# ultravideo/kvazaar

Measured on AMD Instinct MI355X. Metric: CTUs/s (all-intra ultrafast hot path), higher is better.
Workload: dtype u8/i16 (f64 RD costs)

## Files before the change

### include/kvz_hip_dev.h

```cpp
#ifndef KVZ_HIP_DEV_H_
#define KVZ_HIP_DEV_H_

#include "kvz_hip_types.h"

#ifdef __cplusplus
extern "C" {
#endif

void *kvz_hip_dev_alloc(size_t bytes);
void  kvz_hip_dev_free(void *p);
void  kvz_hip_dev_upload(void *dev_dst, const void *host_src, size_t bytes);
void  kvz_hip_dev_download(void *host_dst, const void *dev_src, size_t bytes);
void  kvz_hip_dev_sync(void);
void  kvz_hip_dev_copy(void *dev_dst, const void *dev_src, size_t bytes);
void  kvz_hip_dev_timer_start(void);
float kvz_hip_dev_timer_stop(void);

int  kvz_hip_dev_sad_nxn(int n, const uint8_t *a, const uint8_t *b, int count, uint32_t *out);
int  kvz_hip_dev_satd_nxn(int n, const uint8_t *a, const uint8_t *b, int count, uint32_t *out);

int  kvz_hip_dev_transform(int kind, const int16_t *in, int16_t *tmp, int16_t *out, int count, int use_matrix_cores);

int  kvz_hip_dev_angular_pred(int log2_width, int mode, const uint8_t *ref_above, const uint8_t *ref_left, int count, uint8_t *out);

int  kvz_hip_dev_intra_select(int log2w, int nblk, const uint32_t *raw, const int8_t *preds, const double *mode_bits, int count, int32_t *winner);

void kvz_hip_dev_deblock_frames(uint8_t *frames, int width, int height, int n_frames, const uint8_t *cu_depth, int qp, int beta_offset_div2,
                                int tc_offset_div2);

typedef struct kvz_hip_cu_dbk {
  uint8_t type;
  uint8_t depth, tr_depth, part_size;
  uint8_t cbf_y;
  uint8_t mv_dir;
  int8_t  mv_ref[2];
  int16_t ref_id[2];
  int16_t mv[2][2];
} kvz_hip_cu_dbk;
void kvz_hip_dev_deblock_frames_inter(uint8_t *frames, int width, int height, int n_frames, const kvz_hip_cu_dbk *info, int qp, int beta_offset_div2,
                                      int tc_offset_div2, int slice_is_b);

int  kvz_hip_dev_loop_filters_inter(const uint8_t *src, uint8_t *rec, int width, int height, int n_pictures, const kvz_hip_cu_dbk *info, int qp, int slice_is_b, int deblock,
                                    int beta_offset_div2, int tc_offset_div2, int sao, int no_wpp, kvz_hip_sao_params *luma, kvz_hip_sao_params *chroma, uint8_t *merge);

int  kvz_hip_dev_sad_surface(const uint8_t *cur, const uint8_t *ref, int width, int height, int bw, int range, const int16_t *blk_xy, int count,
                             uint32_t *out);

typedef struct kvz_hip_fme_pu {
// ... 98 lines not shown
```

### kvazaar_amd/csrc/kvz_ctu.hpp

```cpp
#pragma once
#include <type_traits>
#include "../../include/kvz_hip_types.h"
#include "kvz_ops.hpp"
#include "kvz_rdoq.hpp"
#include "kvz_recon.hpp"
#include "kvz_residual.hpp"
#include "kvz_select.hpp"

namespace kvz {

#define KVZ_CTU_THREADS 128
#ifdef KVZ_HOSTSIM
#define KVZ_FOR_THREADS(tid) for (int tid = 0; tid < KVZ_CTU_THREADS; ++tid)
#ifdef KVZ_HOSTSIM_COUNT_SYNCS
static unsigned long long g_kvz_syncs;
#define KVZ_SYNC() (++g_kvz_syncs)
#else
#define KVZ_SYNC()
#endif
#define KVZ_LDS_ADD(p, v) (*(p) += (v))
#else
#define KVZ_FOR_THREADS(tid) for (int tid = (threadIdx.x + lane_rot) & (KVZ_CTU_THREADS - 1), once_ = 1; once_; once_ = 0)
#define KVZ_SYNC() __syncthreads()
#define KVZ_LDS_ADD(p, v) atomicAdd((p), (v))
#endif
#ifdef KVZ_HOSTSIM
#define KVZ_WAVE_SYNC()
#else
#define KVZ_WAVE_SYNC() do { __builtin_amdgcn_fence(__ATOMIC_RELEASE, "wavefront"); __builtin_amdgcn_wave_barrier(); __builtin_amdgcn_fence(__ATOMIC_ACQUIRE, "wavefront"); } while (0)
#endif

#ifdef KVZ_HOSTSIM
#define KVZ_TOGETHER(...)
#else
#define KVZ_TG1(v) "+v"(v)
#define KVZ_TG_PICK(_1, _2, _3, _4, _5, _6, _7, _8, _9, _10, NAME, ...) NAME
#define KVZ_TG_2(a, b) KVZ_TG1(a), KVZ_TG1(b)
#define KVZ_TG_5(a, b, c, d, e) KVZ_TG1(a), KVZ_TG1(b), KVZ_TG1(c), KVZ_TG1(d), KVZ_TG1(e)
#define KVZ_TG_10(a, b, c, d, e, f, g, h, i, j) KVZ_TG_5(a, b, c, d, e), KVZ_TG_5(f, g, h, i, j)
#define KVZ_TOGETHER(...) asm volatile("" : KVZ_TG_PICK(__VA_ARGS__, KVZ_TG_10, _9, _8, _7, _6, KVZ_TG_5, _4, _3, KVZ_TG_2, _1)(__VA_ARGS__))
#endif

KVZ_DEV void block_add(u32 *dst, u32 v)
{
#ifdef KVZ_HOSTSIM
  *dst += v;
#else
  const int x = row16_sum((int)v);
  const u32 total = (u32)(__builtin_amdgcn_readlane(x, 15) + __builtin_amdgcn_readlane(x, 31) + __builtin_amdgcn_readlane(x, 47) + __builtin_amdgcn_readlane(x, 63));
  if ((threadIdx.x & 63) == 0 && total) atomicAdd(dst, total);
#endif
}
// ... 789 lines not shown
        const int c = g < ny ? 0 : 1, i = g - (c == 0 ? 0 : ny);
        const int l2 = c ? log2w_c : log2w_y, n = 2 * (1 << l2) + 1, side = i >= n, k = side ? i - n : i;
        int qx, qy, dv;
        const bool have = ref_coords(l2, c, x, y, side, k, avail_top, avail_left, &qx, &qy);
        const lds_off off = rec_off(lv, c, qx, qy, &dv);
        s->ref[c][side][k] = have ? base[off] : (u8)128;
        if (c) s->ref[2][side][k] = have ? base[off + dv] : (u8)128;
      }
    }
    KVZ_SYNC();
    KVZ_FOR_THREADS(tid) {
      if (luma) {
        const int n = 2 * (1 << log2w_y) + 1;
        for (int i = tid; i < 2 * n; i += KVZ_CTU_THREADS) {
          const int side = i >= n, k = side ? i - n : i;
          const u8 *r = s->ref[0][side];
          u8 v;
          if (k == 0) v = (u8)((s->ref[0][1][1] + 2 * s->ref[0][1][0] + s->ref[0][0][1] + 2) / 4);
          else if (k == n - 1) v = r[k];
          else v = (u8)((r[k - 1] + 2 * r[k] + r[k + 1] + 2) / 4);
          s->fref[side][k] = v;
        }
      }
      const int c = tid - (KVZ_CTU_THREADS - 3);
      if (c >= 0 && ((c == 0 && luma) || (c > 0 && chroma))) {
        const int l2 = c ? log2w_c : log2w_y, w = 1 << l2;
#ifdef KVZ_HOSTSIM
        s->dcval[c] = (u8)dc_value(l2, s->ref[c][0], s->ref[c][1]);
#else
        u32 sum = 0;
        for (int i = 0; i < w; i += 4) {
          u32 a, b;
          __builtin_memcpy(&a, &s->ref[c][0][1 + i], 4);
          __builtin_memcpy(&b, &s->ref[c][1][1 + i], 4);
          sum = __builtin_amdgcn_sad_u8(a, 0u, sum);
          sum = __builtin_amdgcn_sad_u8(b, 0u, sum);
        }
        s->dcval[c] = (u8)((sum + w) >> (l2 + 1));
#endif
      }
    }
    KVZ_SYNC();
    KVZ_PROF(KVZ_P_REFS);
  }

  KVZ_DEV u8 predict_pixel(int log2w, int mode, int c, int x, int y) const
  {
// ... 504 lines not shown
  KVZ_DEV void transform_big(int l2, i16 *x, bool inverse, int tid, int c) const
  {
#ifndef KVZ_HOSTSIM
    if ((tid >> 6) != (c & 1)) return;
    if (l2 == 5) mfma_transform_block<32>(x, x, inverse, tb, tid & 63);
    else mfma_transform_block<16>(x, x, inverse, tb, tid & 63);
#else
    if (tid != 0) return;
    const int n = 1 << l2;
    i16 tmp[32 * 32];
    for (int pass = 0; pass < 2; pass++) {
      const i16 *src = pass == 0 ? x : tmp;
      i16 *dst = pass == 0 ? tmp : x;
      const int shift = inverse ? (pass == 0 ? 7 : 12) : (pass == 0 ? l2 - 1 : l2 + 6);
      for (int e = 0; e < n * n; e++) {
        const int hi = e >> l2, lo = e & (n - 1);
        dst[e] = inverse ? inv_point(n, [&](int k) { return dct_at(l2, k, lo); }, src, hi, n, shift) : fwd_point(n, [&](int i) { return dct_at(l2, hi, i); }, src, lo << l2, shift);
      }
    }
#endif
  }

  enum RowPlan { ROWS_CU8, ROWS_W16, ROWS_W32_Y, ROWS_W32_C };
  KVZ_DEV void plane_sums(RowPlan plan, int tid, int c, u32 v, bool packed, int base) const
  {
#ifdef KVZ_HOSTSIM
    (void)tid;
    if (c < 0) return;
    if (packed && plan != ROWS_CU8) { s->acc[3 + c] += v & 0xffffffu; s->acc[6 + c] += v >> 24; }
    else s->acc[base + c] += v;
#else
    (void)c;
    if ((plan == ROWS_W16 || plan == ROWS_W32_C) && tid >= 64) return;
    const int x = row16_sum((int)v);
    const u32 r0 = (u32)__builtin_amdgcn_readlane(x, 15), r1 = (u32)__builtin_amdgcn_readlane(x, 31), r2 = (u32)__builtin_amdgcn_readlane(x, 47), r3 = (u32)__builtin_amdgcn_readlane(x, 63);
    if ((tid & 63) != 0) return;
    if (plan == ROWS_CU8) {
      if (tid < 64) s->acc[base] += r0 + r1 + r2 + r3;
      else { s->acc[base + 1] += r0; s->acc[base + 2] += r1; }
      return;
    }
    auto put = [&](int plane, u32 a, u32 b) {
      if (packed) {
        const u32 ws = (a & 0xffffffu) + (b & 0xffffffu), n = (a >> 24) + (b >> 24);
        if (n) { atomicAdd(&s->acc[3 + plane], ws); atomicAdd(&s->acc[6 + plane], n); }
        else if (ws) atomicAdd(&s->acc[3 + plane], ws);
      } else if (a + b) atomicAdd(&s->acc[base + plane], a + b);
    };
    if (plan == ROWS_W16) { put(0, r0, r1); put(1, r2, 0); put(2, r3, 0); }
    else if (plan == ROWS_W32_Y) { put(0, r0, r1); put(0, r2, r3); }
    else { put(1, r0, r1); put(2, r2, r3); }
#endif
  }
  KVZ_DEV void finish_planes(int lv, int xl, int yl, int depth, int c0, int c1, bool packed) const
  {
    for (int c = c0; c < c1; c++) {
      u32 n = s->acc[6 + c];
      if (packed) { const u32 pk = s->acc[3 + c]; n = pk >> 24; s->acc[3 + c] = pk & 0xffffffu; s->acc[6 + c] = n; }
      if (NXN && lv == 4) { if (c == 0) rl->pu_cbf[rl->n_pu] = n != 0; else rl->pu_cbf_c[c - 1] = n != 0; }
      else {
        CtuCu *cu = &s->cu[lv][(yl >> 3) * 8 + (xl >> 3)];
        cbf_clear(&cu->cbf, depth, c);
        if (n) cbf_set(&cu->cbf, depth, c);
      }
    }
  }
  KVZ_DEV void hide_signs(int tid, int log2y, int log2c, int scan, const i16 *cf_y, i16 *lv_y, const i16 *cf_u, i16 *lv_u, const i16 *cf_v, i16 *lv_v) const
  {
    if constexpr (SH) {
      const int wv = tid >> 6, lane = tid & 63;
      const int c = wv == 0 ? 0 : 1 + (lane >> 4), i = wv == 0 ? lane : (lane & 15), l2 = wv == 0 ? log2y : log2c, groups = 1 << (2 * l2 - 4);
      const bool live = c < 3 && i < groups;
      const i16 *cf = c == 0 ? cf_y : (c == 1 ? cf_u : cf_v);
      i16 *lv = c == 0 ? lv_y : (c == 1 ? lv_u : lv_v);
// ... 14 lines not shown
      const bool first_visited = ((behind >> i) >> 1) == 0;
#endif
      if (any) {
        auto at = [&](int n) { const int r = scan_in_group(scan, n); return base + ((r >> 2) << l2) + (r & 3); };
        const SignHideChange ch = sign_hide_group([&](int n) { return (int)lv[at(n)]; }, [&](int n) { return (int)cf[at(n)]; }, s->qs[l2 - 2][c ? 1 : 0], first_visited);
        if (ch.pos >= 0) { const int o = at(ch.pos); lv[o] = (i16)sign_hide_apply(lv[o], cf[o], ch.step); }
      }
    }
  }
  KVZ_DEV void recon_cu8(int lv, const TuSet &t, int depth, int mode)
  {
    const int xl = t.x - cx, yl = t.y - cy;
    const CandView cv = cand_view(lv);
#define KVZ_CU8_STAGE(body) KVZ_FOR_THREADS(tid) { if (tid < 64) { body(std::true_type(), tid); } else if (tid < 96) { body(std::false_type(), tid); } }
#define KVZ_CU8_ROLE(tid)                                                                                               \
    constexpr bool LUMA = decltype(luma)::value;                                                                        \
    constexpr int l2 = LUMA ? 3 : 2, n = 1 << l2, sh = LUMA ? 0 : 1;                                                    \
    const int c = LUMA ? 0 : ((tid) < 80 ? 1 : 2), e = LUMA ? (tid) : ((tid) & 15);                                     \
    (void)sh; (void)n; (void)c; (void)e
    KVZ_FOR_THREADS(tid) {
      if (tid < 2) s->acc[3 * tid] = 0;
      if (tid >= 64 && tid < 68) s->acc[1 + (tid - 64) + ((tid - 64) >> 1)] = 0;
    }
    auto stage1 = [&](auto luma, int tid) {
      KVZ_CU8_ROLE(tid);
      const int px = e & (n - 1), py = e >> l2;
      const u8 p = predict_pixel(l2, mode, c, px, py);
      cv.at(c, (xl >> sh) + px, (yl >> sh) + py) = p;
      tbuf(t, 0, c)[e] = (i16)((int)*org_at(c, (xl >> sh) + px, (yl >> sh) + py) - (int)p);
    };
    KVZ_CU8_STAGE(stage1)
    KVZ_WAVE_SYNC();
    KVZ_PROF(KVZ_P_RPRED);
    auto stage2 = [&](auto luma, int tid) {
      KVZ_CU8_ROLE(tid);
      const int k = e >> l2, j = e & (n - 1);
      constexpr int shift = l2 - 1, add = 1 << (shift - 1);
      const i16 *src = tbuf(t, 0, c);
      int a = 0;
#pragma unroll
      for (int i = 0; i < n; i++) a += dct_at(l2, k, i) * (int)src[(j << l2) + i];
      tbuf(t, 1, c)[e] = (i16)((a + add) >> shift);
    };
    KVZ_CU8_STAGE(stage2)
    KVZ_WAVE_SYNC();
    KVZ_PROF(KVZ_P_FDCT);
    const bool hide = hide_on();
    KVZ_FOR_THREADS(tid) {
      u32 packed = 0;
      auto stage3 = [&](auto luma, int tid_) {
        KVZ_CU8_ROLE(tid_);
        const int k = e >> l2, j = e & (n - 1);
        constexpr int shift = l2 + 6, add = 1 << (shift - 1);
        const i16 *src = tbuf(t, 1, c);
        int a = 0;
#pragma unroll
        for (int i = 0; i < n; i++) a += dct_at(l2, k, i) * (int)src[(j << l2) + i];
        const int cf = (i16)((a + add) >> shift);
        const QuantScalars q = s->qs[l2 - 2][LUMA ? 0 : 1];
        ListFactor f{ 0, 0 };
        if constexpr (LISTS) f = factor_at(c, l2, e);
        const int level = LISTS ? quant_level(cf, q, f.fwd) : quant_level(cf, q);
        levels_lds(lv, c)[e] = (i16)level;
        if constexpr (SH) { if (hide) { tbuf(t, 0, c)[e] = (i16)cf; return; } }
        tbuf(t, 0, c)[e] = LISTS ? dequant_level(level, q, f.inv) : dequant_level(level, q);
        packed = level_cost(level, m->coeff_weights).word();
      };
      if (tid < 64) stage3(std::true_type(), tid); else if (tid < 96) stage3(std::false_type(), tid);
      if (!hide) plane_sums(ROWS_CU8, tid, tid < 64 ? 0 : (tid < 80 ? 1 : (tid < 96 ? 2 : -1)), packed, true, 3);
    }
    if constexpr (SH) {
      if (hide) {
        KVZ_WAVE_SYNC();
        KVZ_FOR_THREADS(tid) { hide_signs(tid, 3, 2, intra_scan_order(mode, depth), tbuf(t, 0, 0), levels_lds(lv, 0), tbuf(t, 0, 1), levels_lds(lv, 1), tbuf(t, 0, 2), levels_lds(lv, 2)); }
        KVZ_WAVE_SYNC();
        KVZ_FOR_THREADS(tid) {
          u32 packed = 0;
          auto stage3b = [&](auto luma, int tid_) {
            KVZ_CU8_ROLE(tid_);
            const int level = levels_lds(lv, c)[e];
            tbuf(t, 0, c)[e] = dequant_level(level, s->qs[l2 - 2][LUMA ? 0 : 1]);
            packed = level_cost(level, m->coeff_weights).word();
          };
          if (tid < 64) stage3b(std::true_type(), tid); else if (tid < 96) stage3b(std::false_type(), tid);
          plane_sums(ROWS_CU8, tid, tid < 64 ? 0 : (tid < 80 ? 1 : (tid < 96 ? 2 : -1)), packed, true, 3);
        }
      }
    }
    KVZ_WAVE_SYNC();
    KVZ_PROF(KVZ_P_QUANT);
    auto stage4 = [&](auto luma, int tid) {
      KVZ_CU8_ROLE(tid);
      if (s->acc[3 + c] >> 24) {
        const int j = e >> l2, i = e & (n - 1);
        constexpr int shift = 7, add = 1 << (shift - 1);
        const i16 *src = tbuf(t, 0, c);
        int a = 0;
#pragma unroll
        for (int k = 0; k < n; k++) a += dct_at(l2, k, i) * (int)src[(k << l2) + j];
        tbuf(t, 1, c)[e] = (i16)iclip(-32768, 32767, (a + add) >> shift);
      }
    };
    KVZ_CU8_STAGE(stage4)
    KVZ_WAVE_SYNC();
    KVZ_PROF(KVZ_P_IDCT);
    KVZ_FOR_THREADS(tid) {
      u32 ssd = 0;
      auto stage5 = [&](auto luma, int tid_) {
        KVZ_CU8_ROLE(tid_);
        u8 *rp = &cv.at(c, (xl >> sh) + (e & (n - 1)), (yl >> sh) + (e >> l2));
        int v = *rp;
        if (s->acc[3 + c] >> 24) {
          const int j = e >> l2, i = e & (n - 1);
          constexpr int shift = 12, add = 1 << (shift - 1);
          const i16 *src = tbuf(t, 1, c);
          int a = 0;
#pragma unroll
          for (int k = 0; k < n; k++) a += dct_at(l2, k, i) * (int)src[(k << l2) + j];
          const i16 res = (i16)iclip(-32768, 32767, (a + add) >> shift);
          v = recon_sample(v, res);
          *rp = (u8)v;
        }
        ssd = sq_err(*org_at(c, (xl >> sh) + (e & (n - 1)), (yl >> sh) + (e >> l2)), v);
      };
      if (tid < 64) stage5(std::true_type(), tid); else if (tid < 96) stage5(std::false_type(), tid);
      plane_sums(ROWS_CU8, tid, tid < 64 ? 0 : (tid < 80 ? 1 : (tid < 96 ? 2 : -1)), ssd, false, 0);
    }
    KVZ_SYNC();
    KVZ_FOR_THREADS(tid) {
      if (tid == 0) finish_planes(lv, xl, yl, depth, 0, 3, true);
    }
    if (cabac_on()) KVZ_SYNC();
    KVZ_PROF(KVZ_P_RECON);
#undef KVZ_CU8_ROLE
#undef KVZ_CU8_STAGE
  }

  KVZ_DEV void rdoq_unit(int tid, int lv, const TuSet &t, bool chroma, int depth, int mode) const
  {
#ifdef KVZ_HOSTSIM
    const int wv = tid == 0 ? 0 : (tid == 64 ? 1 : -1), lane = 0;
#else
    const int wv = tid >> 6, lane = tid & 63;
#endif
    for (int c = 0; c < (chroma ? 3 : 1); c++) {
      if (wv != (c ? 1 : 0)) continue;
      RdoqWaveArgs ra;
      ra.ptab = (KVZ_LDS_PTR(const i32))rl->ptab; ra.coef = (KVZ_LDS_PTR(const i16))tbuf(t, 0, c); ra.dest = (KVZ_LDS_PTR(i16))levels_lds(lv, c);
      ra.diag8 = (KVZ_LDS_PTR(const u8))rl->diag8; ra.lambda = m->lambda; ra.qp = m->qp; ra.log2w = tu_log2(t, c); ra.type = c ? 2 : 0;
      ra.scan_mode = intra_scan_order(mode, depth);
// ... 1368 lines not shown
```

### kvazaar_amd/csrc/kvz_dev.hpp

```cpp
#pragma once
#include <hip/hip_runtime.h>

#include <functional>
#include <mutex>
#include <chrono>
#include <vector>

#include "../../include/kvz_hip_dev.h"
#include "kvz_mfma.hpp"
#include "kvz_ops.hpp"
#include "kvz_sao.hpp"
#include "kvz_entropy.hpp"
#include "kvz_select.hpp"

namespace kvz {

__device__ __forceinline__ u32 load_u32_any(const u8 *p) { u32 v; __builtin_memcpy(&v, p, 4); return v; }
template <int G> __device__ __forceinline__ u32 group_sum(u32 v)
{
  for (int off = G / 2; off > 0; off >>= 1) v += __shfl_down(v, off, G);
  return v;
}

template <int N> __global__ void __launch_bounds__(256) dev_sad_kernel(const uint4 *a, const uint4 *b, const long chunks, u32 *out)
{
  constexpr int G = N * N / 16;
  const long i = (long)blockIdx.x * 256 + threadIdx.x;
  u32 v = 0;
  if (i < chunks) {
    const uint4 x = a[i], y = b[i];
    v = __builtin_amdgcn_sad_u8(x.x, y.x, 0);
    v = __builtin_amdgcn_sad_u8(x.y, y.y, v);
    v = __builtin_amdgcn_sad_u8(x.z, y.z, v);
    v = __builtin_amdgcn_sad_u8(x.w, y.w, v);
  }
  if (G <= 64) {
// ... 206 lines not shown
    dev_product<16>(v, Tt, sTt, false, lane, 64, t);
    for (int r = 0; r < 4; r++) v[r] = iclip(-32768, 32767, t[r] >> 7);
    dev_product<16>(v, Tt, sTt, false, lane, 2048, t);
    for (int r = 0; r < 4; r++) v[r] = iclip(-32768, 32767, t[r] >> 12);
  }
  for (int r = 0; r < 4; r++) {
    const int row = M::row(lane, r);
    if (have && row / NB == g) o[(row - g * NB) * NB + cc] = (i16)v[r];
  }
}

constexpr int kAngularGroupsPerLane = 8;
__global__ void __launch_bounds__(256) dev_intra_select_kernel(const u32 *raw, const int8_t *preds, const double *mode_bits, const int count, const int log2w, const int nblk,
                                                               int32_t *winner)
{
  const long table = (long)blockIdx.x * 4 + (threadIdx.x >> 6);
  if (table >= count) return;
  const int lane = threadIdx.x & 63, my_mode = lane < 35 ? lane : 0;
  const int p0 = preds[3 * table], p1 = preds[3 * table + 1], p2 = preds[3 * table + 2];
  const double bits[3] = { mode_bits[3 * table], mode_bits[3 * table + 1], mode_bits[3 * table + 2] };
  const u32 my_raw = select_satd_sum(raw + (table * 35 + my_mode) * nblk, nblk);
  const int w = select_on_wave(lane, my_raw, select_mode_cost(my_raw, my_mode, p0, p1, p2, bits), p0, p1, p2, log2w);
  if (lane == 0) winner[table] = w;
}

template <int L2> __global__ void __launch_bounds__(256) dev_angular_kernel(const u8 *above, const u8 *left, const int count, const int mode, u8 *out)
{
  constexpr int W = 1 << L2, NG = kAngularGroupsPerLane, GPB = W * W / 4, BLOCKS = 256 * NG / GPB, RS = 2 * W + 1, ES = (2 * W + 1 + 8 + 3) & ~3;
  constexpr int RAW = (BLOCKS * RS + 3 + 3) / 4 + 2;
  __shared__ u32 s_raw[2][RAW];
  __shared__ alignas(8) u8 s_ext[BLOCKS][ES];
  __shared__ u32 s_tile[BLOCKS * W * W / 4];
  const int disp_tab[9] = { 0, 2, 5, 9, 13, 17, 21, 26, 32 };
  const int inv_tab[9] = { 0, 4096, 1638, 910, 630, 482, 390, 315, 256 };
  const bool vertical = mode >= 18;
  const int mode_disp = vertical ? mode - 26 : 10 - mode, ad = iabs(mode_disp);
  const int disp = mode_disp < 0 ? -disp_tab[ad] : disp_tab[ad], inv = inv_tab[ad];
  const long blk0 = (long)blockIdx.x * BLOCKS;
  const int nblk = (int)(count - blk0 < BLOCKS ? count - blk0 : BLOCKS);
  const long g0 = blk0 * RS;
  const int mis = (int)(g0 & 3), ndw = (mis + nblk * RS + 3) >> 2;
  const u8 *main_g = vertical ? above : left, *side_g = vertical ? left : above;
  const int tid = threadIdx.x;
  for (int i = tid; i < ndw; i += 256) {
    s_raw[0][i] = reinterpret_cast<const u32 *>(main_g + g0 - mis)[i];
    if (disp < 0) s_raw[1][i] = reinterpret_cast<const u32 *>(side_g + g0 - mis)[i];
// ... 835 lines not shown
  return 0;
}

int kvz_hip_dev_angular_pred(int log2_width, int mode, const uint8_t *ref_above, const uint8_t *ref_left, int count, uint8_t *out)
{
  if (count <= 0) return 0;
  const int blocks_per_wg = 256 * kvz::kAngularGroupsPerLane / ((1 << (2 * log2_width)) / 4);
  const long threads = ((long)count + blocks_per_wg - 1) / blocks_per_wg * 256;
  switch (log2_width) {
  case 2: KVZ_DEV_LAUNCH(kvz::dev_angular_kernel<2>, threads, ref_above, ref_left, count, mode, out); break;
  case 3: KVZ_DEV_LAUNCH(kvz::dev_angular_kernel<3>, threads, ref_above, ref_left, count, mode, out); break;
  case 4: KVZ_DEV_LAUNCH(kvz::dev_angular_kernel<4>, threads, ref_above, ref_left, count, mode, out); break;
  case 5: KVZ_DEV_LAUNCH(kvz::dev_angular_kernel<5>, threads, ref_above, ref_left, count, mode, out); break;
  default: fprintf(stderr, "kvz_hip_dev_angular_pred: unsupported log2_width=%d\n", log2_width); return -1;
  }
  return 0;
}

int kvz_hip_dev_intra_select(int log2w, int nblk, const uint32_t *raw, const int8_t *preds, const double *mode_bits, int count, int32_t *winner)
{
  if (!((log2w == 3 && nblk == 1) || (log2w == 4 && nblk == 4))) { fprintf(stderr, "kvz_hip_dev_intra_select: unsupported log2w=%d nblk=%d\n", log2w, nblk); return -1; }
  if (count <= 0) return 0;
  KVZ_DEV_LAUNCH(kvz::dev_intra_select_kernel, ((long)count + 3) / 4 * 256, raw, preds, mode_bits, count, log2w, nblk, winner);
  return 0;
}

void kvz_hip_dev_deblock_frames(uint8_t *frames, int width, int height, int n_frames, const uint8_t *cu_depth, int qp, int beta_offset_div2,
                                int tc_offset_div2)
{
  kvz::deblock_frames_on(be().stream, frames, width, height, n_frames, cu_depth, qp, beta_offset_div2, tc_offset_div2);
}

void kvz_hip_dev_deblock_frames_inter(uint8_t *frames, int width, int height, int n_frames, const kvz_hip_cu_dbk *info, int qp, int beta_offset_div2, int tc_offset_div2,
                                      int slice_is_b)
{
  kvz::deblock_frames_on(be().stream, frames, width, height, n_frames, nullptr, qp, beta_offset_div2, tc_offset_div2, 3, info, slice_is_b);
}

namespace kvz {
struct LoopScratch {
  u8 *ver = nullptr, *dbk = nullptr; size_t pic_bytes = 0;
  SaoStats *stats = nullptr; SaoCand *cand = nullptr; SaoRec *recs = nullptr; u8 *merge = nullptr; size_t lcus = 0;
  float *fbits = nullptr;
  int32_t *qps = nullptr; size_t n_qps = 0;
  SaoQpRow *sao_rows = nullptr;
};
// ... 831 lines not shown
```

### kvazaar_amd/csrc/kvz_fme.hpp

```cpp
#pragma once
#include <hip/hip_runtime.h>

#include "../../include/kvz_hip_dev.h"
#include "kvz_ops.hpp"
#include "kvz_tables.hpp"

namespace kvz {

template <int MAXN> __global__ void __launch_bounds__(256) dev_fme_kernel(const u8 *cur, const u8 *ref, const int W, const int H, const kvz_hip_fme_pu *pus, const int steps,
                                                                         const Tables *tb, u32 *out)
{
  constexpr int WS = MAXN + 8;
  __shared__ alignas(8) u8 s_win[(MAXN + 8) * WS];
  __shared__ i16 s_g[(MAXN + 8) * (MAXN + 1)];
  __shared__ alignas(8) u8 s_cur[MAXN * MAXN];
  __shared__ alignas(8) u8 s_pred[4][MAXN * MAXN];
  __shared__ u32 s_cost[4];
  const kvz_hip_fme_pu pu = pus[blockIdx.x];
  const int w = pu.w, h = pu.h, tid = threadIdx.x;
  u32 *o = out + (long)blockIdx.x * KVZ_HIP_FME_COSTS;
  if (w > MAXN || h > MAXN) return;
  const int X0 = pu.x + pu.mv_x - 4, Y0 = pu.y + pu.mv_y - 4;
  for (int i = tid; i < (h + 8) * (w + 8); i += 256) {
    const int r = i / (w + 8), c = i - r * (w + 8);
// ... 85 lines not shown
      }
      __syncthreads();
      for (int i = tid; i < wr * w; i += 256) {
        const int r = i / w, c = i - r * w;
        int t = 0;
        for (int k = 0; k < taps; k++) t += hf[k] * (int)s_win[r * WS + c + k];
        s_g[r * MAXN + c] = (i16)t;
      }
      __syncthreads();
      for (int i = tid; i < w * h; i += 256) {
        const int y = i / w, x = i - y * w;
        int t = 0;
        for (int k = 0; k < taps; k++) t += vf[k] * (int)s_g[(y + k) * MAXN + x];
        const int v = t >> 6;
        if (lists == 1) pred[poff + (long)((pu.y >> sh) + y) * fw + (pu.x >> sh) + x] = clip_pixel((v + 32) >> 6);
        else if (first) s_acc[i] = (i16)v;
        else pred[poff + (long)((pu.y >> sh) + y) * fw + (pu.x >> sh) + x] = clip_pixel(((int)s_acc[i] + (int)(i16)v + 64) >> 7);
      }
      first = false;
    }
  }
}

typedef short kvz_short2 __attribute__((ext_vector_type(2)));
KVZ_DEV int dot4_i8(int a, int b, int c) { return __builtin_amdgcn_sdot4(a, b, c, false); }
KVZ_DEV int dot2_i16(unsigned a, unsigned b, int c)
{
  kvz_short2 va, vb;
  __builtin_memcpy(&va, &a, 4); __builtin_memcpy(&vb, &b, 4);
  return __builtin_amdgcn_sdot2(va, vb, c, false);
}
struct McWaveLds {
  alignas(16) u8 win[23 * 32];
  alignas(16) i16 gT[16 * 24];
};

__global__ void __launch_bounds__(256) dev_inter_pred_wave_kernel(const u8 *ref0, const u8 *ref1, u8 *pred, const int W, const int H, const kvz_hip_mc_pu *pus, const int count,
                                                                  const Tables *tb)
{
  __shared__ McWaveLds lds_all[4];
  const int wave = threadIdx.x >> 6, lane = threadIdx.x & 63, pi = blockIdx.x * 4 + wave;
  if (pi >= count) return;
  McWaveLds &L = lds_all[wave];
  const kvz_hip_mc_pu pu = pus[pi];
  const int lists = (pu.use[0] != 0) + (pu.use[1] != 0);
  if (pu.w > 16 || pu.h > 16 || lists == 0) return;
  for (int pass = 0; pass < 2; pass++) {
    const int sh = pass, fw = W >> sh, fh = H >> sh, w = pu.w >> sh, h = pu.h >> sh, taps = pass ? 4 : 8, before = pass ? 1 : 3;
    const int half = pass ? lane >> 5 : 0, hl = pass ? lane & 31 : lane, nl = pass ? 32 : 64;
    const long poff = pass == 0 ? 0 : (half == 0 ? (long)W * H : (long)W * H * 5 / 4);
    const int wstride = pass ? 16 : 32, gstride = pass ? 12 : 24;
    u8 *win = L.win + (pass ? half * 11 * 16 : 0);
    i16 *gT = L.gT + (pass ? half * 8 * 12 : 0);
    int acc0[4] = { 0, 0, 0, 0 };
// ... 89 lines not shown
```

### kvazaar_amd/csrc/kvz_ops.hpp

```cpp
#pragma once
#include <stdint.h>

#ifdef KVZ_HOSTSIM
#define KVZ_DEV inline
#define KVZ_ATOMIC_ADD(p, v) (*(p) += (v))
#else
#include <hip/hip_runtime.h>
#define KVZ_DEV __device__ __forceinline__
#define KVZ_ATOMIC_ADD(p, v) atomicAdd((p), (v))
#endif

namespace kvz {

typedef uint8_t u8;
typedef int16_t i16;
typedef uint16_t u16;
typedef uint32_t u32;
typedef int32_t i32;

#ifdef KVZ_HOSTSIM
#define KVZ_HD inline
#else
#define KVZ_HD __host__ __device__ __forceinline__
#endif
KVZ_HD int iabs(int v) { return v < 0 ? -v : v; }
KVZ_HD int iclip(int lo, int hi, int v) { return v < lo ? lo : (v > hi ? hi : v); }
KVZ_HD int imin(int a, int b) { return a < b ? a : b; }
KVZ_HD int imax(int a, int b) { return a > b ? a : b; }
KVZ_DEV u8 clip_pixel(int v) { return (u8)(v < 0 ? 0 : (v > 255 ? 255 : v)); }
#ifndef KVZ_HOSTSIM
KVZ_DEV int row16_sum(int v)
{
  v += __builtin_amdgcn_update_dpp(0, v, 0x118, 0xF, 0xF, true);
  v += __builtin_amdgcn_update_dpp(0, v, 0x114, 0xF, 0xF, true);
  v += __builtin_amdgcn_update_dpp(0, v, 0x112, 0xF, 0xF, true);
  v += __builtin_amdgcn_update_dpp(0, v, 0x111, 0xF, 0xF, true);
  return v;
}
#endif

constexpr unsigned kMrefStride = 36, kMrefOrg = 16, kMrefRefRow = 68, kMrefFiltered = 408;

struct Tables {
  i16 dct[4][32 * 32];
  i16 dst4[16];
  alignas(16) int8_t dct_i8[2][2][32 * 32];
  alignas(16) i32 dct_sum[2][2][32];
  alignas(16) int8_t bd_i8[3][2][16 * 16];
  alignas(16) i32 bd_sum[3][2][16];
  u32 small_pairs[3][2][8][4];
  u32 pairs16[2][16][8];
  u32 scan[3][4][1024];
// ... 598 lines not shown
```

### kvazaar_amd/csrc/kvz_recon.hpp

```cpp
#pragma once
#include "kvz_ops.hpp"
#include "kvz_syntax.hpp"

namespace kvz {

KVZ_HD bool luma_reads_filtered(int log2w, int mode)
{
  if (mode == 1 || log2w == 2) return false;
  return mode == 0 || imin(iabs(mode - 26), iabs(mode - 10)) > (log2w == 3 ? 7 : (log2w == 4 ? 1 : 0));
}

template <class Mat> KVZ_DEV i16 fwd_point(int n, Mat m, const i16 *in, int at, int shift)
{
  int a = 0;
  for (int i = 0; i < n; i++) a += m(i) * (int)in[at + i];
  return (i16)((a + (1 << (shift - 1))) >> shift);
}
template <class Mat> KVZ_DEV i16 inv_point(int n, Mat m, const i16 *in, int at, int stride, int shift)
{
  int a = 0;
  for (int k = 0; k < n; k++) a += m(k) * (int)in[k * stride + at];
  return (i16)iclip(-32768, 32767, (a + (1 << (shift - 1))) >> shift);
}

KVZ_HD int quant_level(int cf, const QuantScalars &q, int fwd)
{
  int level = (int)(((u32)iabs(cf) * (u32)fwd + (u32)q.add) >> q.q_bits);
  if (cf < 0) level = -level;
  return iclip(-32768, 32767, level);
}
KVZ_HD int quant_level(int cf, const QuantScalars &q) { return quant_level(cf, q, q.flat_q); }

KVZ_HD int quant_delta_u(int cf, int level, const QuantScalars &q)
{
  return (int)((u32)iabs(cf) * (u32)q.flat_q - ((u32)iabs(level) << q.q_bits)) >> (q.q_bits - 8);
}
struct SignHideChange { int pos, step; };
template <class LevelAt, class CoeffAt> KVZ_HD SignHideChange sign_hide_group(LevelAt level_at, CoeffAt coeff_at, const QuantScalars &q, bool first_visited)
{
  int first_nz = 16, last_nz = -1, sum = 0;
  for (int n = 0; n < 16; n++) {
    const int l = level_at(n);
    if (l) { if (first_nz == 16) first_nz = n; last_nz = n; }
    sum += l;
  }
  SignHideChange best{ -1, 0 };
// ... 80 lines not shown
```

### kvazaar_amd/dev.py

```python
import ctypes as C

import numpy as np

TRANSFORM_KINDS = {"dct4": 0, "dct8": 1, "dct16": 2, "dct32": 3, "dst4": 4, "idct4": 5, "idct8": 6, "idct16": 7, "idct32": 8, "idst4": 9}
TRANSFORM_SIZE = {0: 4, 1: 8, 2: 16, 3: 32, 4: 4, 5: 4, 6: 8, 7: 16, 8: 32, 9: 4}


class Dev:
    def __init__(self, cdll):
        self.lib = l = cdll
        vp, sz, ci = C.c_void_p, C.c_size_t, C.c_int
        l.kvz_hip_dev_alloc.restype = vp; l.kvz_hip_dev_alloc.argtypes = [sz]
        l.kvz_hip_dev_free.restype = None; l.kvz_hip_dev_free.argtypes = [vp]
        l.kvz_hip_dev_upload.restype = None; l.kvz_hip_dev_upload.argtypes = [vp, vp, sz]
        l.kvz_hip_dev_download.restype = None; l.kvz_hip_dev_download.argtypes = [vp, vp, sz]
        l.kvz_hip_dev_sync.restype = None; l.kvz_hip_dev_sync.argtypes = []
        l.kvz_hip_dev_timer_start.restype = None; l.kvz_hip_dev_timer_start.argtypes = []
        l.kvz_hip_dev_timer_stop.restype = C.c_float; l.kvz_hip_dev_timer_stop.argtypes = []
        for f in (l.kvz_hip_dev_sad_nxn, l.kvz_hip_dev_satd_nxn):
            f.restype = None; f.argtypes = [ci, vp, vp, ci, vp]
        l.kvz_hip_dev_transform.restype = None; l.kvz_hip_dev_transform.argtypes = [ci, vp, vp, vp, ci, ci]
        l.kvz_hip_dev_angular_pred.restype = None; l.kvz_hip_dev_angular_pred.argtypes = [ci, ci, vp, vp, ci, vp]
        l.kvz_hip_dev_intra_select.restype = ci; l.kvz_hip_dev_intra_select.argtypes = [ci, ci, vp, vp, vp, ci, vp]

    def put(self, a):
        a = np.ascontiguousarray(a)
        p = self.lib.kvz_hip_dev_alloc(a.nbytes)
        self.lib.kvz_hip_dev_upload(p, a.ctypes.data, a.nbytes)
        return p

    def copy_in(self, p, a):
        a = np.ascontiguousarray(a)
        self.lib.kvz_hip_dev_upload(p, a.ctypes.data, a.nbytes)

    def empty(self, nbytes):
        return self.lib.kvz_hip_dev_alloc(nbytes)

    def get(self, p, shape, dtype):
        out = np.empty(shape, dtype)
        self.lib.kvz_hip_dev_download(out.ctypes.data, p, out.nbytes)
        return out

    def free(self, *ps):
        for p in ps:
            self.lib.kvz_hip_dev_free(p)
```

Baseline: 2.927 million.

## Use packed dot2 row transforms with transposed LDS layout in CU8 recon

Rewrites the CU8 intra transform stages so each lane preloads its forward and inverse matrix rows into registers and computes the butterfly-free DCT with packed 16-bit dot2 instructions over contiguous LDS rows. Intermediates are stored transposed so each lane reads a contiguous aligned row. The change also keeps prediction/original samples and the coded flag in registers instead of re-reading LDS and the shared accumulator. It adds a standalone test kernel and entry point, and uses more registers per lane, which may lower occupancy.

```diff
diff --git a/include/kvz_hip_dev.h b/include/kvz_hip_dev.h
--- a/include/kvz_hip_dev.h
+++ b/include/kvz_hip_dev.h
@@ -24,6 +24,8 @@
 int  kvz_hip_dev_angular_pred(int log2_width, int mode, const uint8_t *ref_above, const uint8_t *ref_left, int count, uint8_t *out);
 
 int  kvz_hip_dev_intra_select(int log2w, int nblk, const uint32_t *raw, const int8_t *preds, const double *mode_bits, int count, int32_t *winner);
+
+int  kvz_hip_dev_cu8_units(int count, int from_coeffs, const int16_t *in, const int32_t *qp, int16_t *levels, int16_t *dequant, int16_t *resid);
 
 void kvz_hip_dev_deblock_frames(uint8_t *frames, int width, int height, int n_frames, const uint8_t *cu_depth, int qp, int beta_offset_div2,
                                 int tc_offset_div2);
diff --git a/kvazaar_amd/csrc/kvz_ctu.hpp b/kvazaar_amd/csrc/kvz_ctu.hpp
--- a/kvazaar_amd/csrc/kvz_ctu.hpp
+++ b/kvazaar_amd/csrc/kvz_ctu.hpp
@@ -28,6 +28,14 @@
 #define KVZ_WAVE_SYNC()
 #else
 #define KVZ_WAVE_SYNC() do { __builtin_amdgcn_fence(__ATOMIC_RELEASE, "wavefront"); __builtin_amdgcn_wave_barrier(); __builtin_amdgcn_fence(__ATOMIC_ACQUIRE, "wavefront"); } while (0)
+#endif
+
+#ifdef KVZ_HOSTSIM
+#define KVZ_LANE_VAR(type, name) type name[KVZ_CTU_THREADS] = {}
+#define KVZ_LANE(name, tid) name[tid]
+#else
+#define KVZ_LANE_VAR(type, name) type name = {}
+#define KVZ_LANE(name, tid) name
 #endif
 
 #ifdef KVZ_HOSTSIM
@@ -863,7 +871,7 @@
           s->fref[side][k] = v;
         }
       }
-      const int c = tid - (KVZ_CTU_THREADS - 3);
+      const int c = mover_lane(tid) - (KVZ_CTU_THREADS - 3);
       if (c >= 0 && ((c == 0 && luma) || (c > 0 && chroma))) {
         const int l2 = c ? log2w_c : log2w_y, w = 1 << l2;
 #ifdef KVZ_HOSTSIM
@@ -1414,24 +1422,28 @@
   }
 
   enum RowPlan { ROWS_CU8, ROWS_W16, ROWS_W32_Y, ROWS_W32_C };
-  KVZ_DEV void plane_sums(RowPlan plan, int tid, int c, u32 v, bool packed, int base) const
+  KVZ_DEV u32 plane_sums(RowPlan plan, int tid, int c, u32 v, bool packed, int base) const
   {
 #ifdef KVZ_HOSTSIM
     (void)tid;
-    if (c < 0) return;
+    if (c < 0) return 0;
     if (packed && plan != ROWS_CU8) { s->acc[3 + c] += v & 0xffffffu; s->acc[6 + c] += v >> 24; }
     else s->acc[base + c] += v;
+    return 0;
 #else
     (void)c;
-    if ((plan == ROWS_W16 || plan == ROWS_W32_C) && tid >= 64) return;
+    if ((plan == ROWS_W16 || plan == ROWS_W32_C) && tid >= 64) return 0;
     const int x = row16_sum((int)v);
     const u32 r0 = (u32)__builtin_amdgcn_readlane(x, 15), r1 = (u32)__builtin_amdgcn_readlane(x, 31), r2 = (u32)__builtin_amdgcn_readlane(x, 47), r3 = (u32)__builtin_amdgcn_readlane(x, 63);
-    if ((tid & 63) != 0) return;
     if (plan == ROWS_CU8) {
-      if (tid < 64) s->acc[base] += r0 + r1 + r2 + r3;
-      else { s->acc[base + 1] += r0; s->acc[base + 2] += r1; }
-      return;
-    }
+      const u32 luma = r0 + r1 + r2 + r3;
+      if ((tid & 63) == 0) {
+        if (tid < 64) s->acc[base] += luma;
+        else { s->acc[base + 1] += r0; s->acc[base + 2] += r1; }
+      }
+      return tid < 64 ? luma : (tid < 80 ? r0 : r1);
+    }
+    if ((tid & 63) != 0) return 0;
     auto put = [&](int plane, u32 a, u32 b) {
       if (packed) {
         const u32 ws = (a & 0xffffffu) + (b & 0xffffffu), n = (a >> 24) + (b >> 24);
@@ -1442,6 +1454,7 @@
     if (plan == ROWS_W16) { put(0, r0, r1); put(1, r2, 0); put(2, r3, 0); }
     else if (plan == ROWS_W32_Y) { put(0, r0, r1); put(0, r2, r3); }
     else { put(1, r0, r1); put(2, r2, r3); }
+    return 0;
 #endif
   }
   KVZ_DEV void finish_planes(int lv, int xl, int yl, int depth, int c0, int c1, bool packed) const
@@ -1502,25 +1515,26 @@
       if (tid < 2) s->acc[3 * tid] = 0;
       if (tid >= 64 && tid < 68) s->acc[1 + (tid - 64) + ((tid - 64) >> 1)] = 0;
     }
+    KVZ_LANE_VAR(WideBytes<16>, mat_f);
+    KVZ_LANE_VAR(WideBytes<16>, mat_i);
+    KVZ_LANE_VAR(u32, pred_org);
+    KVZ_LANE_VAR(u32, plane_word);
     auto stage1 = [&](auto luma, int tid) {
       KVZ_CU8_ROLE(tid);
       const int px = e & (n - 1), py = e >> l2;
+      cu8_matrix_rows<l2>(tb, e, KVZ_LANE(mat_f, tid), KVZ_LANE(mat_i, tid));
       const u8 p = predict_pixel(l2, mode, c, px, py);
       cv.at(c, (xl >> sh) + px, (yl >> sh) + py) = p;
-      tbuf(t, 0, c)[e] = (i16)((int)*org_at(c, (xl >> sh) + px, (yl >> sh) + py) - (int)p);
+      const u8 o = *org_at(c, (xl >> sh) + px, (yl >> sh) + py);
+      KVZ_LANE(pred_org, tid) = (u32)p | ((u32)o << 8);
+      tbuf(t, 0, c)[e] = (i16)((int)o - (int)p);
     };
     KVZ_CU8_STAGE(stage1)
     KVZ_WAVE_SYNC();
     KVZ_PROF(KVZ_P_RPRED);
     auto stage2 = [&](auto luma, int tid) {
       KVZ_CU8_ROLE(tid);
-      const int k = e >> l2, j = e & (n - 1);
-      constexpr int shift = l2 - 1, add = 1 << (shift - 1);
-      const i16 *src = tbuf(t, 0, c);
-      int a = 0;
-#pragma unroll
-      for (int i = 0; i < n; i++) a += dct_at(l2, k, i) * (int)src[(j << l2) + i];
-      tbuf(t, 1, c)[e] = (i16)((a + add) >> shift);
+      tbuf(t, 1, c)[e] = cu8_fwd_first<l2>(tbuf(t, 0, c), e, KVZ_LANE(mat_f, tid));
     };
     KVZ_CU8_STAGE(stage2)
     KVZ_WAVE_SYNC();
@@ -1530,24 +1544,18 @@
       u32 packed = 0;
       auto stage3 = [&](auto luma, int tid_) {
         KVZ_CU8_ROLE(tid_);
-        const int k = e >> l2, j = e & (n - 1);
-        constexpr int shift = l2 + 6, add = 1 << (shift - 1);
-        const i16 *src = tbuf(t, 1, c);
-        int a = 0;
-#pragma unroll
-        for (int i = 0; i < n; i++) a += dct_at(l2, k, i) * (int)src[(j << l2) + i];
-        const int cf = (i16)((a + add) >> shift);
+        const int cf = cu8_fwd_second<l2>(tbuf(t, 1, c), e, KVZ_LANE(mat_f, tid_));
         const QuantScalars q = s->qs[l2 - 2][LUMA ? 0 : 1];
         ListFactor f{ 0, 0 };
         if constexpr (LISTS) f = factor_at(c, l2, e);
         const int level = LISTS ? quant_level(cf, q, f.fwd) : quant_level(cf, q);
         levels_lds(lv, c)[e] = (i16)level;
         if constexpr (SH) { if (hide) { tbuf(t, 0, c)[e] = (i16)cf; return; } }
-        tbuf(t, 0, c)[e] = LISTS ? dequant_level(level, q, f.inv) : dequant_level(level, q);
+        tbuf(t, 0, c)[cu8_transposed<l2>(e)] = LISTS ? dequant_level(level, q, f.inv) : dequant_level(level, q);
         packed = level_cost(level, m->coeff_weights).word();
       };
       if (tid < 64) stage3(std::true_type(), tid); else if (tid < 96) stage3(std::false_type(), tid);
-      if (!hide) plane_sums(ROWS_CU8, tid, tid < 64 ? 0 : (tid < 80 ? 1 : (tid < 96 ? 2 : -1)), packed, true, 3);
+      if (!hide) KVZ_LANE(plane_word, tid) = plane_sums(ROWS_CU8, tid, tid < 64 ? 0 : (tid < 80 ? 1 : (tid < 96 ? 2 : -1)), packed, true, 3);
     }
     if constexpr (SH) {
       if (hide) {
@@ -1559,26 +1567,25 @@
           auto stage3b = [&](auto luma, int tid_) {
             KVZ_CU8_ROLE(tid_);
             const int level = levels_lds(lv, c)[e];
-            tbuf(t, 0, c)[e] = dequant_level(level, s->qs[l2 - 2][LUMA ? 0 : 1]);
+            tbuf(t, 0, c)[cu8_transposed<l2>(e)] = dequant_level(level, s->qs[l2 - 2][LUMA ? 0 : 1]);
             packed = level_cost(level, m->coeff_weights).word();
           };
           if (tid < 64) stage3b(std::true_type(), tid); else if (tid < 96) stage3b(std::false_type(), tid);
-          plane_sums(ROWS_CU8, tid, tid < 64 ? 0 : (tid < 80 ? 1 : (tid < 96 ? 2 : -1)), packed, true, 3);
+          KVZ_LANE(plane_word, tid) = plane_sums(ROWS_CU8, tid, tid < 64 ? 0 : (tid < 80 ? 1 : (tid < 96 ? 2 : -1)), packed, true, 3);
         }
       }
     }
     KVZ_WAVE_SYNC();
     KVZ_PROF(KVZ_P_QUANT);
+#ifdef KVZ_HOSTSIM
+#define KVZ_CU8_CODED(tid) ((void)KVZ_LANE(plane_word, tid), (s->acc[3 + c] >> 24) != 0)
+#else
+#define KVZ_CU8_CODED(tid) ((KVZ_LANE(plane_word, tid) >> 24) != 0)
+#endif
     auto stage4 = [&](auto luma, int tid) {
       KVZ_CU8_ROLE(tid);
-      if (s->acc[3 + c] >> 24) {
-        const int j = e >> l2, i = e & (n - 1);
-        constexpr int shift = 7, add = 1 << (shift - 1);
-        const i16 *src = tbuf(t, 0, c);
-        int a = 0;
-#pragma unroll
-        for (int k = 0; k < n; k++) a += dct_at(l2, k, i) * (int)src[(k << l2) + j];
-        tbuf(t, 1, c)[e] = (i16)iclip(-32768, 32767, (a + add) >> shift);
+      if (KVZ_CU8_CODED(tid)) {
+        tbuf(t, 1, c)[cu8_transposed<l2>(e)] = cu8_inv_first<l2>(tbuf(t, 0, c), e, KVZ_LANE(mat_i, tid));
       }
     };
     KVZ_CU8_STAGE(stage4)
@@ -1588,24 +1595,17 @@
       u32 ssd = 0;
       auto stage5 = [&](auto luma, int tid_) {
         KVZ_CU8_ROLE(tid_);
-        u8 *rp = &cv.at(c, (xl >> sh) + (e & (n - 1)), (yl >> sh) + (e >> l2));
-        int v = *rp;
-        if (s->acc[3 + c] >> 24) {
-          const int j = e >> l2, i = e & (n - 1);
-          constexpr int shift = 12, add = 1 << (shift - 1);
-          const i16 *src = tbuf(t, 1, c);
-          int a = 0;
-#pragma unroll
-          for (int k = 0; k < n; k++) a += dct_at(l2, k, i) * (int)src[(k << l2) + j];
-          const i16 res = (i16)iclip(-32768, 32767, (a + add) >> shift);
-          v = recon_sample(v, res);
-          *rp = (u8)v;
-        }
-        ssd = sq_err(*org_at(c, (xl >> sh) + (e & (n - 1)), (yl >> sh) + (e >> l2)), v);
+        int v = (int)(KVZ_LANE(pred_org, tid_) & 0xffu);
+        if (KVZ_CU8_CODED(tid_)) {
+          v = recon_sample(v, cu8_inv_second<l2>(tbuf(t, 1, c), e, KVZ_LANE(mat_i, tid_)));
+          cv.at(c, (xl >> sh) + (e & (n - 1)), (yl >> sh) + (e >> l2)) = (u8)v;
+        }
+        ssd = sq_err((int)(KVZ_LANE(pred_org, tid_) >> 8), v);
       };
       if (tid < 64) stage5(std::true_type(), tid); else if (tid < 96) stage5(std::false_type(), tid);
       plane_sums(ROWS_CU8, tid, tid < 64 ? 0 : (tid < 80 ? 1 : (tid < 96 ? 2 : -1)), ssd, false, 0);
     }
+#undef KVZ_CU8_CODED
     KVZ_SYNC();
     KVZ_FOR_THREADS(tid) {
       if (tid == 0) finish_planes(lv, xl, yl, depth, 0, 3, true);
diff --git a/kvazaar_amd/csrc/kvz_dev.hpp b/kvazaar_amd/csrc/kvz_dev.hpp
--- a/kvazaar_amd/csrc/kvz_dev.hpp
+++ b/kvazaar_amd/csrc/kvz_dev.hpp
@@ -12,6 +12,8 @@
 #include "kvz_sao.hpp"
 #include "kvz_entropy.hpp"
 #include "kvz_select.hpp"
+#include "kvz_recon.hpp"
+#include "kvz_tables.hpp"
 
 namespace kvz {
 
@@ -264,6 +266,46 @@
   const u32 my_raw = select_satd_sum(raw + (table * 35 + my_mode) * nblk, nblk);
   const int w = select_on_wave(lane, my_raw, select_mode_cost(my_raw, my_mode, p0, p1, p2, bits), p0, p1, p2, log2w);
   if (lane == 0) winner[table] = w;
+}
+
+struct Cu8MatRow { u32 w[4]; };
+template <int L2> KVZ_DEV void dev_cu8_lane(int stage, int c, int e, i16 (*t)[96], int from_coeffs, int qp, const Cu8MatRow &fwd, const Cu8MatRow &inv, const i16 *in, i16 *levels, i16 *dequant,
+                                            i16 *resid)
+{
+  const int po = c == 0 ? 0 : (c == 1 ? 64 : 80);
+  i16 *t0 = t[0] + po, *t1 = t[1] + po;
+  if (stage == 1) { if (!from_coeffs) t0[e] = in[po + e]; }
+  else if (stage == 2) { if (!from_coeffs) t1[e] = cu8_fwd_first<L2>(t0, e, fwd); }
+  else if (stage == 3) {
+    int level = 0, dq = in[po + e];
+    if (!from_coeffs) {
+      const QuantScalars q = quant_scalars(qp, 8, 1, 0, 1 << L2, c ? 2 : 0);
+      level = quant_level(cu8_fwd_second<L2>(t1, e, fwd), q);
+      dq = dequant_level(level, q);
+    }
+    levels[po + e] = (i16)level;
+    dequant[po + e] = (i16)dq;
+    t0[cu8_transposed<L2>(e)] = (i16)dq;
+  }
+  else if (stage == 4) t1[cu8_transposed<L2>(e)] = cu8_inv_first<L2>(t0, e, inv);
+  else resid[po + e] = cu8_inv_second<L2>(t1, e, inv);
+}
+__global__ void __launch_bounds__(256) dev_cu8_units_kernel(const i16 *in, const int32_t *qp, const int count, const int from_coeffs, const Tables *tb, i16 *levels, i16 *dequant, i16 *resid)
+{
+  __shared__ alignas(16) i16 t[2][2][96];
+  const int half = threadIdx.x >> 7, tid = threadIdx.x & 127;
+  const long unit = 2l * blockIdx.x + half, o = 96 * unit;
+  const bool live = unit < count && tid < 96;
+  const int c = tid < 64 ? 0 : (tid < 80 ? 1 : 2), e = tid < 64 ? tid : (tid & 15), q = live ? qp[unit] : 0;
+  Cu8MatRow fwd = {}, inv = {};
+  if (tid < 64) cu8_matrix_rows<3>(tb, e, fwd, inv); else cu8_matrix_rows<2>(tb, e, fwd, inv);
+  for (int stage = 1; stage <= 5; stage++) {
+    if (live) {
+      if (tid < 64) dev_cu8_lane<3>(stage, c, e, t[half], from_coeffs, q, fwd, inv, in + o, levels + o, dequant + o, resid + o);
+      else dev_cu8_lane<2>(stage, c, e, t[half], from_coeffs, q, fwd, inv, in + o, levels + o, dequant + o, resid + o);
+    }
+    __syncthreads();
+  }
 }
 
 template <int L2> __global__ void __launch_bounds__(256) dev_angular_kernel(const u8 *above, const u8 *left, const int count, const int mode, u8 *out)
@@ -1145,6 +1187,14 @@
   if (!((log2w == 3 && nblk == 1) || (log2w == 4 && nblk == 4))) { fprintf(stderr, "kvz_hip_dev_intra_select: unsupported log2w=%d nblk=%d\n", log2w, nblk); return -1; }
   if (count <= 0) return 0;
   KVZ_DEV_LAUNCH(kvz::dev_intra_select_kernel, ((long)count + 3) / 4 * 256, raw, preds, mode_bits, count, log2w, nblk, winner);
+  return 0;
+}
+
+int kvz_hip_dev_cu8_units(int count, int from_coeffs, const int16_t *in, const int32_t *qp, int16_t *levels, int16_t *dequant, int16_t *resid)
+{
+  if (count < 0 || (from_coeffs != 0 && from_coeffs != 1)) { fprintf(stderr, "kvz_hip_dev_cu8_units: count=%d from_coeffs=%d\n", count, from_coeffs); return -1; }
+  if (count == 0) return 0;
+  KVZ_DEV_LAUNCH(kvz::dev_cu8_units_kernel, ((long)count + 1) / 2 * 256, in, qp, count, from_coeffs, kvz::device_tables(), levels, dequant, resid);
   return 0;
 }
 
diff --git a/kvazaar_amd/csrc/kvz_fme.hpp b/kvazaar_amd/csrc/kvz_fme.hpp
--- a/kvazaar_amd/csrc/kvz_fme.hpp
+++ b/kvazaar_amd/csrc/kvz_fme.hpp
@@ -131,14 +131,7 @@
   }
 }
 
-typedef short kvz_short2 __attribute__((ext_vector_type(2)));
 KVZ_DEV int dot4_i8(int a, int b, int c) { return __builtin_amdgcn_sdot4(a, b, c, false); }
-KVZ_DEV int dot2_i16(unsigned a, unsigned b, int c)
-{
-  kvz_short2 va, vb;
-  __builtin_memcpy(&va, &a, 4); __builtin_memcpy(&vb, &b, 4);
-  return __builtin_amdgcn_sdot2(va, vb, c, false);
-}
 struct McWaveLds {
   alignas(16) u8 win[23 * 32];
   alignas(16) i16 gT[16 * 24];
diff --git a/kvazaar_amd/csrc/kvz_ops.hpp b/kvazaar_amd/csrc/kvz_ops.hpp
--- a/kvazaar_amd/csrc/kvz_ops.hpp
+++ b/kvazaar_amd/csrc/kvz_ops.hpp
@@ -28,6 +28,17 @@
 KVZ_HD int imin(int a, int b) { return a < b ? a : b; }
 KVZ_HD int imax(int a, int b) { return a > b ? a : b; }
 KVZ_DEV u8 clip_pixel(int v) { return (u8)(v < 0 ? 0 : (v > 255 ? 255 : v)); }
+#ifdef KVZ_HOSTSIM
+KVZ_DEV int dot2_i16(unsigned a, unsigned b, int c) { return c + (int)(i16)(a & 0xffffu) * (int)(i16)(b & 0xffffu) + (int)(i16)(a >> 16) * (int)(i16)(b >> 16); }
+#else
+typedef short kvz_short2 __attribute__((ext_vector_type(2)));
+KVZ_DEV int dot2_i16(unsigned a, unsigned b, int c)
+{
+  kvz_short2 va, vb;
+  __builtin_memcpy(&va, &a, 4); __builtin_memcpy(&vb, &b, 4);
+  return __builtin_amdgcn_sdot2(va, vb, c, false);
+}
+#endif
 #ifndef KVZ_HOSTSIM
 KVZ_DEV int row16_sum(int v)
 {
diff --git a/kvazaar_amd/csrc/kvz_recon.hpp b/kvazaar_amd/csrc/kvz_recon.hpp
--- a/kvazaar_amd/csrc/kvz_recon.hpp
+++ b/kvazaar_amd/csrc/kvz_recon.hpp
@@ -22,6 +22,41 @@
   for (int k = 0; k < n; k++) a += m(k) * (int)in[k * stride + at];
   return (i16)iclip(-32768, 32767, (a + (1 << (shift - 1))) >> shift);
 }
+
+template <int N, class Row, class MatRow> KVZ_DEV int row_dot(const Row &x, const MatRow &m)
+{
+  int a = 0;
+  for (int i = 0; i < N / 2; i++) a = dot2_i16(x.w[i], m.w[i], a);
+  return a;
+}
+template <int N, class Row, class MatRow> KVZ_DEV i16 fwd_row_point(const Row &x, const MatRow &m, int shift) { return (i16)((row_dot<N>(x, m) + (1 << (shift - 1))) >> shift); }
+template <int N, class Row, class MatRow> KVZ_DEV i16 inv_row_point(const Row &x, const MatRow &m, int shift)
+{
+  return (i16)iclip(-32768, 32767, (row_dot<N>(x, m) + (1 << (shift - 1))) >> shift);
+}
+
+template <int N> struct alignas(2 * N) Int16Row { u32 w[N / 2]; };
+template <int N> KVZ_DEV Int16Row<N> int16_row(const i16 *p)
+{
+  Int16Row<N> r;
+#ifdef KVZ_HOSTSIM
+  __builtin_memcpy(&r, p, 2 * N);
+#else
+  __builtin_memcpy(&r, __builtin_assume_aligned(p, 2 * N), 2 * N);
+#endif
+  return r;
+}
+template <int L2> KVZ_HD int cu8_transposed(int e) { return ((e & ((1 << L2) - 1)) << L2) + (e >> L2); }
+template <int L2, class MatRow> KVZ_DEV void cu8_matrix_rows(const Tables *tb, int e, MatRow &fwd, MatRow &inv)
+{
+  constexpr int n = 1 << L2;
+  __builtin_memcpy(&fwd, &tb->small_pairs[L2 == 3 ? 1 : 0][0][e >> L2][0], 2 * n);
+  __builtin_memcpy(&inv, &tb->small_pairs[L2 == 3 ? 1 : 0][1][e & (n - 1)][0], 2 * n);
+}
+template <int L2, class MatRow> KVZ_DEV i16 cu8_fwd_first(const i16 *t0, int e, const MatRow &fwd) { return fwd_row_point<(1 << L2)>(int16_row<(1 << L2)>(t0 + ((e & ((1 << L2) - 1)) << L2)), fwd, L2 - 1); }
+template <int L2, class MatRow> KVZ_DEV i16 cu8_fwd_second(const i16 *t1, int e, const MatRow &fwd) { return fwd_row_point<(1 << L2)>(int16_row<(1 << L2)>(t1 + ((e & ((1 << L2) - 1)) << L2)), fwd, L2 + 6); }
+template <int L2, class MatRow> KVZ_DEV i16 cu8_inv_first(const i16 *t0, int e, const MatRow &inv) { return inv_row_point<(1 << L2)>(int16_row<(1 << L2)>(t0 + ((e >> L2) << L2)), inv, 7); }
+template <int L2, class MatRow> KVZ_DEV i16 cu8_inv_second(const i16 *t1, int e, const MatRow &inv) { return inv_row_point<(1 << L2)>(int16_row<(1 << L2)>(t1 + ((e >> L2) << L2)), inv, 12); }
 
 KVZ_HD int quant_level(int cf, const QuantScalars &q, int fwd)
 {
diff --git a/kvazaar_amd/dev.py b/kvazaar_amd/dev.py
--- a/kvazaar_amd/dev.py
+++ b/kvazaar_amd/dev.py
@@ -22,6 +22,7 @@
         l.kvz_hip_dev_transform.restype = None; l.kvz_hip_dev_transform.argtypes = [ci, vp, vp, vp, ci, ci]
         l.kvz_hip_dev_angular_pred.restype = None; l.kvz_hip_dev_angular_pred.argtypes = [ci, ci, vp, vp, ci, vp]
         l.kvz_hip_dev_intra_select.restype = ci; l.kvz_hip_dev_intra_select.argtypes = [ci, ci, vp, vp, vp, ci, vp]
+        l.kvz_hip_dev_cu8_units.restype = ci; l.kvz_hip_dev_cu8_units.argtypes = [ci, ci, vp, vp, vp, vp, vp]
 
     def put(self, a):
         a = np.ascontiguousarray(a)
```

Result: faster. 3.062 million (median of 6 runs) (+4.6%).
